# xUhEngwAng/I2V-Adapter-Unofficial

Measured on AMD Instinct MI355X. Metric: denoising steps/sec @ 16fx512x512 SD1.5+I2V-Adapter, higher is better.
Workload: dtype f16

## Files before the change

i2v-adapter-unofficial_amd/_lib.py:

```python
import ctypes as C
import os

_HERE = os.path.dirname(os.path.abspath(__file__))
LIB_PATH = os.environ.get("I2V_LIB_PATH") or os.path.join(_HERE, "libi2v_hip.so")
ABI_VERSION = 28

I2V_EPI_NONE, I2V_EPI_GELU, I2V_EPI_GEGLU = 0, 1, 2
I2V_STORE_ROWMAJOR, I2V_STORE_ROWPERM, I2V_STORE_VT, I2V_STORE_VT_T = 0, 1, 2, 3
I2V_A_PLAIN, I2V_A_CONV3X3 = 0, 1
I2V_LORA_MAX_ADAPTERS, I2V_LORA_MAX_RANK = 8, 256
I2V_ROUTE_GENERIC, I2V_ROUTE_CONV_THIN, I2V_ROUTE_BIG_TILE, I2V_ROUTE_BIG_DEEP, I2V_ROUTE_BIG_SPLITK = 0, 1, 2, 3, 4
I2V_EXTRA_NONE, I2V_EXTRA_LNF, I2V_EXTRA_HILO, I2V_EXTRA_GNS, I2V_EXTRA_UPF = 0, 1, 2, 4, 8
I2V_TATTN_LDS_FORM, I2V_TATTN_REG_FORM = 0, 1
I2V_ADD_RES_MAX = 16
I2V_TAESD_PREP_IDENTITY, I2V_TAESD_PREP_UNIT, I2V_TAESD_PREP_CLAMP = 0, 1, 2


class HipLibraryError(RuntimeError):
    pass


class GemmParams(C.Structure):
    _fields_ = [
        ("a", C.c_void_p), ("lda", C.c_int64),
        ("a2", C.c_void_p), ("lda2", C.c_int64),
        ("k_split", C.c_int32), ("a_mode", C.c_int32),
        ("w", C.c_void_p), ("ldw", C.c_int64),
        ("bias", C.c_void_p),
# ... 223 lines not shown
    "i2v_gemm_f16": (C.c_int, [C.POINTER(GemmParams), _P]),
    "i2v_gemm_ln_supported": (C.c_int, [C.POINTER(GemmParams)]),
    "i2v_gemm_batch_supported": (C.c_int, [C.POINTER(GemmParams)]),
    "i2v_gemm_upconv_fold_supported": (C.c_int, [C.POINTER(GemmParams)]),
    "i2v_gemm_workspace_bytes": (C.c_int64, [C.POINTER(GemmParams)]),
    "i2v_gemm_gn_partial_rows": (C.c_int32, [C.POINTER(GemmParams)]),
    "i2v_gemm_route": (C.c_int, [C.POINTER(GemmParams), C.POINTER(GemmRoute)]),
    "i2v_gemm_last_route": (C.c_int, [C.POINTER(GemmRoute)]),
    "i2v_gemm_kernel_exists": (C.c_int, [C.POINTER(GemmRoute)]),
    "i2v_attention_f16": (C.c_int, [C.POINTER(AttnParams), _P]),
    "i2v_temporal_attention_f16": (C.c_int, [C.POINTER(TAttnParams), _P]),
    "i2v_temporal_attention_route": (C.c_int, [C.POINTER(TAttnParams), C.POINTER(TAttnRoute)]),
    "i2v_temporal_attention_last_route": (C.c_int, [C.POINTER(TAttnRoute)]),
    "i2v_tattn_kernel_exists": (C.c_int, [C.POINTER(TAttnRoute)]),
    "i2v_motion_attn_supported": (C.c_int32, [C.c_int64, C.c_int32, C.c_int32, C.c_int32, C.c_int32]),
    "i2v_motion_attn_pack_rows": (C.c_int32, [C.c_int32, C.c_int32]),
    "i2v_motion_attn_f16": (C.c_int, [C.POINTER(MotionAttnParams), _P]),
    "i2v_motion_attn_wide_supported": (C.c_int32, [C.c_int64, C.c_int32, C.c_int32, C.c_int32, C.c_int32]),
    "i2v_motion_attn_wide_f16": (C.c_int, [C.POINTER(MotionAttnParams), _P]),
    "i2v_cross_attn_fused_supported": (C.c_int32, [C.c_int64, C.c_int32, C.c_int32, C.c_int32, C.c_int32, C.c_int64]),
    "i2v_cross_attn_fused_pack_rows": (C.c_int32, [C.c_int32, C.c_int32]),
    "i2v_cross_attn_fused_ctx_elems": (C.c_int64, [C.c_int32, C.c_int32, C.c_int32]),
    "i2v_cross_attn_fused_f16": (C.c_int, [C.POINTER(CrossAttnFusedParams), _P]),
    "i2v_ln_qkv_supported": (C.c_int32, [C.c_int64, C.c_int32, C.c_int32, C.c_int64]),
    "i2v_ln_qkv_f16": (C.c_int, [C.POINTER(LnQkvParams), _P]),
    "i2v_ff_fused_supported": (C.c_int32, [C.c_int64, C.c_int32, C.c_int32]),
    "i2v_ff_fused_tail_supported": (C.c_int32, [C.c_int64, C.c_int32, C.c_int32, C.c_int32, C.c_int32]),
    "i2v_ff_fused_f16": (C.c_int, [C.POINTER(FfFusedParams), _P]),
    "i2v_groupnorm_workspace_bytes": (C.c_int64, [C.c_int32, C.c_int32, C.c_int32]),
    "i2v_groupnorm_f16": (C.c_int, [C.POINTER(GnParams), _P]),
    "i2v_groupnorm_fold_f16": (C.c_int, [C.POINTER(GnParams), _P, C.c_int64, _P, C.c_int32, _P, _P, _P]),
    "i2v_layernorm_f16": (C.c_int, [C.POINTER(LnParams), _P]),
    "i2v_softmax_rows_f16": (C.c_int, [_P, C.c_int64, _P, C.c_int64, C.c_int32, C.c_int32, C.c_float, _P]),
    "i2v_nchw_to_tokens": (C.c_int, [_P, C.c_int32, _P, C.c_int32, C.c_int32, C.c_int32, C.c_int32, _P]),
    "i2v_tokens_to_nchw": (C.c_int, [_P, C.c_int32, C.c_int64, _P, C.c_int32, C.c_int32, C.c_int32, C.c_int32, _P]),
    "i2v_timestep_embedding": (C.c_int, [_P, _P, C.c_int32, _P, C.c_int32, C.c_int32, _P]),
    "i2v_silu_f16": (C.c_int, [_P, _P, C.c_int64, _P]),
    "i2v_repeat_rows_f16": (C.c_int, [_P, _P, C.c_int64, C.c_int64, C.c_int32, _P]),
    "i2v_copy3d_f16": (C.c_int, [_P, C.c_int64, C.c_int64, _P, C.c_int64, C.c_int64, C.c_int64, C.c_int64,
                                 C.c_int64, _P]),
    "i2v_pack_ctx_fragments_elems": (C.c_int64, [C.c_int32, C.c_int32, C.c_int32]),
    "i2v_pack_ctx_fragments_f16": (C.c_int, [_P, C.c_int64, _P, C.c_int64, C.c_int64, _P, C.c_int32, C.c_int32, C.c_int32, C.c_int32, _P]),
    "i2v_ddim_prep": (C.c_int, [_P, _P, _P, C.c_int32, C.c_int32, C.c_int32, C.c_int32, C.c_int32, C.c_int32, _P]),
    "i2v_gaussian_sample_f32": (C.c_int, [_P, _P, _P, C.c_int32, C.c_int32, C.c_int32, _P]),
    "i2v_first_frame_prior_f32": (C.c_int, [_P, _P, _P, _P, C.c_int32, C.c_int32, C.c_int32, C.c_int32, C.c_int32,
                                            C.c_float, C.c_float, C.c_float, C.c_float, C.c_float, _P]),
# ... 120 lines not shown
```

i2v-adapter-unofficial_amd/csrc/handle.hip:

```cpp
#include <string.h>

#include <map>
#include <string>
#include <vector>

#include "common.h"

namespace {

constexpr uint32_t PLAN_MAGIC = 0x50563249u;
constexpr uint32_t PLAN_VERSION = 1;
struct PlanHeader {
  uint32_t magic, version, abi, n_ops, n_keys, n_relocs;
  int32_t batch, frames, height, width, ctx_len, has_ip;
  uint64_t arena_bytes;
  uint32_t io_read_mask, reserved;
  uint64_t keys_off, ops_off, relocs_off, payload_off, payload_bytes, total_bytes;
};
struct PlanOp {
  uint32_t entry, payload_off, payload_bytes, reloc_begin, reloc_count, struct_bytes;
};
struct PlanReloc {
  uint32_t offset, kind, index, pad;
  uint64_t addend;
};
enum { RELOC_ARENA = 0, RELOC_WEIGHT = 1, RELOC_IO = 2 };

enum Entry {
  E_GEMM = 0, E_ATTN, E_TATTN, E_MOTION_ATTN, E_CROSS_ATTN_FUSED, E_LN_QKV, E_FF_FUSED, E_GROUPNORM, E_LAYERNORM,
  E_GROUPNORM_FOLD, E_NCHW_TO_TOKENS, E_TOKENS_TO_NCHW, E_TIMESTEP_EMBEDDING, E_SILU, E_REPEAT_ROWS, E_COPY3D, E_SELECT_ROW,
  E_PACK_CTX_FRAGMENTS, E_DDIM_PREP, E_DDIM_CFG_STEP, E_DPM_CFG_STEP, E_FREEU, E_LCM_CFG_STEP, E_FREENOISE_GATHER,
  E_FREENOISE_BLEND, E_MOTION_ATTN_WIDE, E_COUNT
};
struct EntryInfo {
  const char* name;
  uint32_t struct_bytes;
  uint32_t slots;
};
const EntryInfo ENTRIES[E_COUNT] = {
    {"i2v_gemm_f16", sizeof(i2v_gemm_params), 0},
    {"i2v_attention_f16", sizeof(i2v_attn_params), 0},
    {"i2v_temporal_attention_f16", sizeof(i2v_tattn_params), 0},
    {"i2v_motion_attn_f16", sizeof(i2v_motion_attn_params), 0},
    {"i2v_cross_attn_fused_f16", sizeof(i2v_cross_attn_fused_params), 0},
    {"i2v_ln_qkv_f16", sizeof(i2v_ln_qkv_params), 0},
    {"i2v_ff_fused_f16", sizeof(i2v_ff_fused_params), 0},
    {"i2v_groupnorm_f16", sizeof(i2v_gn_params), 0},
    {"i2v_layernorm_f16", sizeof(i2v_ln_params), 0},
    {"i2v_groupnorm_fold_f16", sizeof(i2v_gn_params), 6},
    {"i2v_nchw_to_tokens", 0, 7},
    {"i2v_tokens_to_nchw", 0, 8},
    {"i2v_timestep_embedding", 0, 6},
    {"i2v_silu_f16", 0, 3},
    {"i2v_repeat_rows_f16", 0, 5},
    {"i2v_copy3d_f16", 0, 9},
    {"i2v_select_row_f16", 0, 6},
    {"i2v_pack_ctx_fragments_f16", 0, 10},
    {"i2v_ddim_prep", 0, 9},
    {"i2v_ddim_cfg_step", 0, 13},
    {"i2v_dpm_cfg_step", 0, 14},
    {"i2v_freeu_f16", 0, 13},
    {"i2v_lcm_cfg_step", 0, 15},
    {"i2v_freenoise_gather_f16", 0, 10},
    {"i2v_freenoise_blend_f16", 0, 12},
    {"i2v_motion_attn_wide_f16", sizeof(i2v_motion_attn_params), 0},
};
inline uint32_t pad8(uint32_t n) { return (n + 7u) & ~7u; }

}

struct i2v_unet {
  i2v_unet_config cfg;
  struct weight { const void* ptr; int32_t dtype, ndim; int64_t shape[4]; };
  std::map<std::string, weight> weights;
  uint64_t weights_generation = 0;
  i2v_unet_plan_t plan;
  bool planned = false;
  std::vector<unsigned char> blob;
  std::vector<std::string> keys;
  std::vector<const void*> key_ptr;
  uint64_t bound_generation = ~0ull;
  void* arena = nullptr;
  int64_t arena_bytes = 0;
  hipStream_t capture_stream = nullptr;
  bool capturing = false;
  hipGraph_t graph = nullptr;
  hipGraphExec_t exec = nullptr;

// ... 302 lines not shown
      case E_DPM_CFG_STEP:
        rc = i2v_dpm_cfg_step(reinterpret_cast<float*>(P(0)), reinterpret_cast<float*>(P(1)), P(2), (int32_t)I(3), I(4),
                              reinterpret_cast<const float*>(P(5)), (int32_t)I(6), reinterpret_cast<int32_t*>(P(7)), F(8), (int32_t)I(9),
                              (int32_t)I(10), (int32_t)I(11), (int32_t)I(12), (int32_t)I(13), stream);
        break;
      case E_FREEU:
        rc = i2v_freeu_f16(P(0), P(1), P(2), P(3), P(4), P(5), (int32_t)I(6), (int32_t)I(7), (int32_t)I(8), (int32_t)I(9), (int32_t)I(10), F(11),
                           F(12), stream);
        break;
      case E_LCM_CFG_STEP:
        rc = i2v_lcm_cfg_step(reinterpret_cast<float*>(P(0)), reinterpret_cast<const float*>(P(1)), (int32_t)I(2), P(3), (int32_t)I(4), I(5),
                              reinterpret_cast<const float*>(P(6)), (int32_t)I(7), reinterpret_cast<int32_t*>(P(8)), F(9), (int32_t)I(10),
                              (int32_t)I(11), (int32_t)I(12), (int32_t)I(13), (int32_t)I(14), stream);
        break;
      case E_FREENOISE_GATHER:
        rc = i2v_freenoise_gather_f16(P(0), I(1), P(2), I(3), reinterpret_cast<const int32_t*>(P(4)), I(5), (int32_t)I(6), (int32_t)I(7),
                                      (int32_t)I(8), (int32_t)I(9), stream);
        break;
      case E_FREENOISE_BLEND:
        rc = i2v_freenoise_blend_f16(P(0), I(1), P(2), I(3), reinterpret_cast<const int32_t*>(P(4)), reinterpret_cast<const float*>(P(5)), I(6),
                                     (int32_t)I(7), (int32_t)I(8), (int32_t)I(9), (int32_t)I(10), (int32_t)I(11), stream);
        break;
      case E_MOTION_ATTN_WIDE: rc = i2v_motion_attn_wide_f16(reinterpret_cast<const i2v_motion_attn_params*>(buf), stream); break;
      default: I2V_FAIL(I2V_ERR_UNSUPPORTED, "i2v_unet_forward: launch %u names entry point %u", i, op.entry);
    }
    if (rc != I2V_OK) return rc;
  }
  return I2V_OK;
}

extern "C" int i2v_unet_capture_step(i2v_unet* h, i2v_stream_t stream) {
  I2V_CHECK_ARG(h != nullptr && stream != nullptr, "i2v_unet_capture_step: null handle or the null stream (capture needs a stream of its own)");
  I2V_CHECK_ARG(h->planned, "i2v_unet_capture_step: i2v_unet_plan first");
  I2V_CHECK_ARG(!h->capturing, "i2v_unet_capture_step: a capture is already in progress (i2v_unet_abort_capture discards it)");
  drop_step(h);
  hipStream_t s = reinterpret_cast<hipStream_t>(stream);
  const hipError_t e = hipStreamBeginCapture(s, hipStreamCaptureModeRelaxed);
  if (e != hipSuccess) {
    (void)hipGetLastError();
    I2V_FAIL(I2V_ERR_LAUNCH, "i2v_unet_capture_step: hipStreamBeginCapture: %s", hipGetErrorString(e));
  }
  h->capture_stream = s;
  h->capturing = true;
  return I2V_OK;
}

// ... 30 lines not shown
```

i2v-adapter-unofficial_amd/csrc/motion_attn.hip:

```cpp
#include <stdlib.h>

#include <type_traits>

#include "common.h"

namespace {

__device__ __forceinline__ f32x4 mfma16x16x16(f16x4 a, f16x4 b, f32x4 c) {
  return __builtin_amdgcn_mfma_f32_16x16x16f16(a, b, c, 0, 0, 0);
}

__device__ __forceinline__ void ma_dma16(__amdgpu_buffer_rsrc_t rsrc, f16* lds_wave_base, unsigned voff, unsigned soff) {
  __builtin_amdgcn_raw_ptr_buffer_load_lds(rsrc, (__attribute__((address_space(3))) void*)lds_wave_base, 16, voff, soff, 0, 0);
}
__device__ __forceinline__ int ma_opaque(int v) {
  asm volatile("" : "+v"(v));
  return v;
}

constexpr int MA_PIX = 8;
constexpr int MA_F = 16;
constexpr int MA_PD = 3;
constexpr int MA_AD = 4;

// ... 1 lines not shown
  const void* x; int64_t ldx;
  const void* gamma; const void* shift; int64_t ld_shift;
  const void* w;
  void* out; int64_t ldo;
  float eps;
  const void* ctx_frag;
  int32_t lt; int32_t tiles_per_ctx;
  const void* ip_frag; int32_t ip_len; float ip_scale;
  const void* w_o; const void* b_o;
};

constexpr int MA_KT = 5;

template <int C, int D, int H, bool CROSS, int F = 16, bool OUTP = false, int PIX = MA_PIX>
__global__ __launch_bounds__(64 * H) void motion_attn_kernel(const ma_args p, const float scale_log2, const int ntiles,
                                                             long long* __restrict__ stamps) {
  constexpr int DT = (D + 15) / 16, DP = 16 * DT, KS = C / 32, NJ = C / 64, PARTS = CROSS ? 1 : 3;
  constexpr int RW = PIX * MA_F / H, HALVES = RW / 8;
  static_assert(C % 64 == 0 && H == 8, "one wave per head, 8 lanes x C / 64 chunks per row in the LayerNorm pass");
  static_assert(F == 8 || F == 16 || F == 32, "frames per pixel");
  static_assert(RW % 8 == 0 && PIX % (F == 32 ? 2 : 1) == 0, "whole groups of 8 rows per wave, whole pixels per tile");
  extern __shared__ __attribute__((aligned(16))) f16 panels[];
  const int tid = threadIdx.x, lane = tid & 63, wave = __builtin_amdgcn_readfirstlane(tid >> 6);
  const int g = lane >> 4, l15 = lane & 15, sub = lane & 7;
  const f16* __restrict__ X = reinterpret_cast<const f16*>(p.x);
  const float* __restrict__ gamma = reinterpret_cast<const float*>(p.gamma);
  const float* __restrict__ shift = reinterpret_cast<const float*>(p.shift);
#ifdef I2V_MA_STAMPS
  long long stamp[8];
#define MA_STAMP(k) stamp[k] = __builtin_amdgcn_s_memtime()
#else
#define MA_STAMP(k)
#endif

  auto fetch_rows = [&](const int tile, f16* panel) {
    const f16* base = X + ((int64_t)tile * (PIX * MA_F) + RW * wave) * p.ldx;
    const auto rs = __builtin_amdgcn_make_buffer_rsrc(const_cast<f16*>(base), 0, (int)(((RW - 1) * p.ldx + C) * 2), 0x00020000);
    const int ln = ma_opaque(lane);
    const unsigned voff = (unsigned)(((ln >> 3) * p.ldx + (ln & 7) * 8) * 2);
#pragma unroll
    for (int half = 0; half < HALVES; ++half)
#pragma unroll
      for (int j = 0; j < NJ; ++j)
        ma_dma16(rs, panel + RW * wave * C + (half * NJ + j) * 512, voff, (unsigned)((8 * half * p.ldx + 8 * j * 8) * 2));
  };
  constexpr bool LATE_TABLES = NJ > 5;
  auto normalise_rows = [&](f16* panel) {
    f16x8 xv[HALVES][NJ];
#pragma unroll
    for (int half = 0; half < HALVES; ++half)
#pragma unroll
      for (int j = 0; j < NJ; ++j) xv[half][j] = *reinterpret_cast<const f16x8*>(panel + RW * wave * C + ((half * NJ + j) * 64 + lane) * 8);
    const float* gp = gamma;
    const float* sp = shift;
    asm volatile("" : "+s"(gp), "+s"(sp));
    f32x4 ga[NJ][2];
    if constexpr (!LATE_TABLES) {
#pragma unroll
      for (int j = 0; j < NJ; ++j) {
        ga[j][0] = *reinterpret_cast<const f32x4*>(gp + (sub + 8 * j) * 8);
        ga[j][1] = *reinterpret_cast<const f32x4*>(gp + (sub + 8 * j) * 8 + 4);
      }
    }
#pragma unroll
    for (int half = 0; half < HALVES; ++half) {
      const int row = RW * wave + 8 * half + (lane >> 3);
      const float* sh = sp + (int64_t)((RW * wave + 8 * half + (lane >> 3)) & (F - 1)) * p.ld_shift;
      f32x4 sv[NJ][2];
      if constexpr (!LATE_TABLES) {
#pragma unroll
// ... 18 lines not shown
      for (int j = 0; j < NJ; ++j)
#pragma unroll
        for (int e = 0; e < 8; ++e) {
          v[j][e] -= mean;
          q = fmaf(v[j][e], v[j][e], q);
        }
      q = sum_lanes8(q);
      const float rstd = rsqrtf(q / (float)C + p.eps);
#pragma unroll
      for (int j = 0; j < NJ; ++j) {
        const int ch = sub + 8 * j;
        if constexpr (LATE_TABLES) {
          ga[j][0] = *reinterpret_cast<const f32x4*>(gp + ch * 8);
          ga[j][1] = *reinterpret_cast<const f32x4*>(gp + ch * 8 + 4);
          sv[j][0] = *reinterpret_cast<const f32x4*>(sh + ch * 8);
          sv[j][1] = *reinterpret_cast<const f32x4*>(sh + ch * 8 + 4);
        }
        f16x8 o;
#pragma unroll
        for (int e = 0; e < 8; ++e) o[e] = (f16)fmaf(v[j][e] * rstd, ga[j][e >> 2][e & 3], sv[j][e >> 2][e & 3]);
        *reinterpret_cast<f16x8*>(panel + row * C + ((ch ^ (row & 7)) * 8)) = o;
      }
    }
  };

  const auto rs_w = __builtin_amdgcn_make_buffer_rsrc(const_cast<void*>(p.w), 0, H * PARTS * DP * C * 2, 0x00020000);
  const int w_lane = lane * 16, w_wave = wave * (PARTS * DP * C * 2);
  const int sw = l15 & 7;
  const int swz[2] = {(g ^ sw) * 8, ((4 + g) ^ sw) * 8};
  f32x4 acc[PIX][DT];
  auto zero_init = [](const int, const int) { return f32x4{0.f, 0.f, 0.f, 0.f}; };
  auto no_hook = []() {};
  auto project = [&](const f16* panel, const __amdgpu_buffer_rsrc_t rs, const int wp, auto transposed, auto init, auto hook) {
    constexpr bool TR = decltype(transposed)::value;
    auto ldw = [&](const int s, const int t) {
      return __builtin_bit_cast(f16x8, __builtin_amdgcn_raw_buffer_load_b128(rs, w_lane, wp + (s * DT + t) * 1024, 0));
    };
    const f16* alane = panel + l15 * C;
    f16x8 wf[MA_PD][DT];
#pragma unroll
    for (int pix = 0; pix < PIX; ++pix)
#pragma unroll
      for (int t = 0; t < DT; ++t) acc[pix][t] = init(pix, t);
#pragma unroll
    for (int s = 0; s < MA_PD - 1; ++s)
#pragma unroll
// ... 126 lines not shown
      __builtin_amdgcn_sched_barrier(0);
    }

    f16x4 qh[PIX][DT];
    project(panel, rs_w, w_wave, std::true_type{}, zero_init, no_hook);
#pragma unroll
    for (int pix = 0; pix < PIX; ++pix)
#pragma unroll
      for (int t = 0; t < DT; ++t) qh[pix][t] = to_half(CROSS ? acc[pix][t] * scale_log2 : acc[pix][t]);
    MA_STAMP(3);
    if constexpr (CROSS && OUTP) lds_barrier();

    if constexpr (CROSS) {
      const int ctx = tile / p.tiles_per_ctx;
      const f16* cf = reinterpret_cast<const f16*>(p.ctx_frag) + ((int64_t)ctx * H + wave) * (2 * MA_KT * DT * 256) + lane * 4;
      f16x4 kf[MA_KT][DT], vf[DT][MA_KT];
#pragma unroll
      for (int kt = 0; kt < MA_KT; ++kt)
#pragma unroll
        for (int t = 0; t < DT; ++t) {
          kf[kt][t] = *reinterpret_cast<const f16x4*>(cf + (kt * DT + t) * 256);
          vf[t][kt] = *reinterpret_cast<const f16x4*>(cf + (MA_KT * DT + t * MA_KT + kt) * 256);
        }
      const bool has_ip = p.ip_len > 0;
      f16x4 kfi[DT], vfi[DT];
      if (has_ip) {
        const f16* ci = reinterpret_cast<const f16*>(p.ip_frag) + ((int64_t)ctx * H + wave) * (2 * MA_KT * DT * 256) + lane * 4;
#pragma unroll
        for (int t = 0; t < DT; ++t) {
          kfi[t] = *reinterpret_cast<const f16x4*>(ci + t * 256);
          vfi[t] = *reinterpret_cast<const f16x4*>(ci + (MA_KT * DT + t * MA_KT) * 256);
        }
      }
      MA_STAMP(4);
      MA_STAMP(5);
      f16* __restrict__ O = reinterpret_cast<f16*>(p.out) + (int64_t)tile * (PIX * MA_F) * p.ldo + wave * D;
      const int sln = ma_opaque(lane), sg = sln >> 4, sl15 = sln & 15;
#pragma unroll
      for (int pix = 0; pix < PIX; ++pix) {
        float sv[MA_KT][4];
        float mx = -INFINITY;
#pragma unroll
        for (int kt = 0; kt < MA_KT; ++kt) {
          f32x4 sacc = {0.f, 0.f, 0.f, 0.f};
#pragma unroll
          for (int t = 0; t < DT; ++t) sacc = mfma16x16x16(kf[kt][t], qh[pix][t], sacc);
#pragma unroll
          for (int r = 0; r < 4; ++r) {
            const bool live = (kt < MA_KT - 1 && p.lt > 16 * (MA_KT - 1)) || 16 * kt + 4 * g + r < p.lt;
            sv[kt][r] = live ? sacc[r] : -INFINITY;
            mx = fmaxf(mx, sv[kt][r]);
          }
        }
        mx = lane_xor32_max(lane_xor16_max(mx));
        float ls = 0.f;
#pragma unroll
        for (int kt = 0; kt < MA_KT; ++kt)
#pragma unroll
          for (int r = 0; r < 4; ++r) {
            sv[kt][r] = __builtin_amdgcn_exp2f(sv[kt][r] - mx);
            ls += sv[kt][r];
          }
        ls = lane_xor32_sum(lane_xor16_sum(ls));
        const float inv = 1.0f / ls;
        f16x4 pk[MA_KT];
#pragma unroll
        for (int kt = 0; kt < MA_KT; ++kt) pk[kt] = f16x4{(f16)sv[kt][0], (f16)sv[kt][1], (f16)sv[kt][2], (f16)sv[kt][3]};
        f32x4 ov[DT];
#pragma unroll
        for (int t = 0; t < DT; ++t) {
          f32x4 o = {0.f, 0.f, 0.f, 0.f};
#pragma unroll
          for (int kt = 0; kt < MA_KT; ++kt) o = mfma16x16x16(vf[t][kt], pk[kt], o);
          ov[t] = o * inv;
        }
        if (has_ip) {
          f32x4 sacc = {0.f, 0.f, 0.f, 0.f};
#pragma unroll
          for (int t = 0; t < DT; ++t) sacc = mfma16x16x16(kfi[t], qh[pix][t], sacc);
          float si[4];
          float mi = -INFINITY;
#pragma unroll
          for (int r = 0; r < 4; ++r) {
            si[r] = (4 * g + r < p.ip_len) ? sacc[r] : -INFINITY;
            mi = fmaxf(mi, si[r]);
          }
          mi = lane_xor32_max(lane_xor16_max(mi));
          float li = 0.f;
#pragma unroll
          for (int r = 0; r < 4; ++r) {
            si[r] = __builtin_amdgcn_exp2f(si[r] - mi);
            li += si[r];
          }
          li = lane_xor32_sum(lane_xor16_sum(li));
          const float wi = p.ip_scale / li;
          const f16x4 pi = {(f16)si[0], (f16)si[1], (f16)si[2], (f16)si[3]};
#pragma unroll
          for (int t = 0; t < DT; ++t) ov[t] += mfma16x16x16(vfi[t], pi, f32x4{0.f, 0.f, 0.f, 0.f}) * wi;
        }
// ... 171 lines not shown
  I2V_CHECK_ARG(p.w_o && p.b_o, "i2v_motion_attn_wide_f16: w_o and b_o are required (this form exists only with the out-projection inside)");
  I2V_CHECK_ARG(i2v_motion_attn_wide_supported(p.rows, p.channels, p.heads, p.head_dim, p.frames),
                "i2v_motion_attn_wide_f16: rows %lld channels %d heads %d head_dim %d frames %d is not a fused shape "
                "(i2v_motion_attn_wide_supported)", (long long)p.rows, p.channels, p.heads, p.head_dim, p.frames);
  I2V_CHECK_ARG(p.ldx >= p.channels && p.ldx % 8 == 0 && p.ldo >= p.channels && p.ldo % 8 == 0 && p.ld_shift >= p.channels &&
                p.ld_shift % 4 == 0, "i2v_motion_attn_wide_f16: row strides");
  I2V_CHECK_ARG(i2v_al16(p.x) && i2v_al16(p.gamma) && i2v_al16(p.shift) && i2v_al16(p.w_qkv) && i2v_al16(p.out) && i2v_al16(p.w_o) &&
                i2v_al16(p.b_o), "i2v_motion_attn_wide_f16: pointers must be 16-byte aligned");
  I2V_CHECK_ARG(p.ldx < (1 << 23), "i2v_motion_attn_wide_f16: ldx (%lld) must be below 2^23", (long long)p.ldx);
  ma_args a = {};
  a.x = p.x; a.ldx = p.ldx; a.gamma = p.gamma; a.shift = p.shift; a.ld_shift = p.ld_shift; a.w = p.w_qkv; a.out = p.out;
  a.ldo = p.ldo; a.eps = p.eps; a.w_o = p.w_o; a.b_o = p.b_o;
  return launch_ma<640, 80, 8, false, 16, true, MA_WIDE_PIX>(a, p.rows, p.scale, reinterpret_cast<hipStream_t>(stream),
                                                              "i2v_motion_attn_wide_f16");
}

extern "C" int32_t i2v_cross_attn_fused_supported(int64_t rows, int32_t channels, int32_t heads, int32_t head_dim, int32_t ctx_len,
                                                  int64_t rows_per_ctx) {
  return rows > 0 && rows % (MA_PIX * MA_F) == 0 && rows / (MA_PIX * MA_F) < (1 << 24) && channels == 320 && heads == 8 &&
         head_dim == 40 && ctx_len >= 1 && ctx_len <= 16 * MA_KT && rows_per_ctx > 0 && rows_per_ctx % (MA_PIX * MA_F) == 0 &&
         rows % rows_per_ctx == 0 && ma_cus<320, 40, 8, true>() > 0;
}

extern "C" int32_t i2v_cross_attn_fused_pack_rows(int32_t heads, int32_t head_dim) { return heads * ((head_dim + 15) / 16) * 16; }

extern "C" int64_t i2v_cross_attn_fused_ctx_elems(int32_t n_ctx, int32_t heads, int32_t head_dim) {
  return (int64_t)n_ctx * heads * 2 * MA_KT * ((head_dim + 15) / 16) * 256;
}

extern "C" int i2v_cross_attn_fused_f16(const i2v_cross_attn_fused_params* pp, i2v_stream_t stream) {
  I2V_CHECK_ARG(pp != nullptr, "i2v_cross_attn_fused_f16: null params");
  const i2v_cross_attn_fused_params& p = *pp;
  I2V_CHECK_ARG(p.x && p.gamma && p.beta && p.w_q && p.ctx_frag && p.out, "i2v_cross_attn_fused_f16: null pointer");
  I2V_CHECK_ARG(i2v_cross_attn_fused_supported(p.rows, p.channels, p.heads, p.head_dim, p.ctx_len, p.rows_per_ctx),
                "i2v_cross_attn_fused_f16: rows %lld channels %d heads %d head_dim %d ctx_len %d rows_per_ctx %lld is not a fused shape "
                "(i2v_cross_attn_fused_supported)", (long long)p.rows, p.channels, p.heads, p.head_dim, p.ctx_len,
                (long long)p.rows_per_ctx);
  I2V_CHECK_ARG(p.ldx >= p.channels && p.ldx % 8 == 0 && p.ldo >= p.channels && p.ldo % 8 == 0, "i2v_cross_attn_fused_f16: row strides");
  I2V_CHECK_ARG(i2v_al16(p.x) && i2v_al16(p.gamma) && i2v_al16(p.beta) && i2v_al16(p.w_q) && i2v_al16(p.out) && i2v_al16(p.ctx_frag) && i2v_al16(p.ip_frag),
                "i2v_cross_attn_fused_f16: pointers must be 16-byte aligned");
  I2V_CHECK_ARG(p.ip_frag == nullptr || (p.ip_len >= 1 && p.ip_len <= 16), "i2v_cross_attn_fused_f16: ip_len (%d) must be in [1, 16]",
                p.ip_len);
  ma_args a = {};
  a.x = p.x; a.ldx = p.ldx; a.gamma = p.gamma; a.shift = p.beta; a.ld_shift = 0; a.w = p.w_q; a.out = p.out; a.ldo = p.ldo;
  a.eps = p.eps;
  a.ctx_frag = p.ctx_frag; a.lt = p.ctx_len;
  a.ip_frag = p.ip_frag; a.ip_len = p.ip_frag ? p.ip_len : 0; a.ip_scale = p.ip_scale;
  a.tiles_per_ctx = (int32_t)(p.rows_per_ctx / (MA_PIX * MA_F));
  I2V_CHECK_ARG(p.w_o == nullptr || p.ldx < (1 << 23), "i2v_cross_attn_fused_f16: ldx (%lld) must be below 2^23 with the out-projection", (long long)p.ldx);
  I2V_CHECK_ARG((p.w_o == nullptr) == (p.b_o == nullptr) && i2v_al16(p.w_o) && i2v_al16(p.b_o),
                "i2v_cross_attn_fused_f16: w_o and b_o come together, 16-byte aligned");
  a.w_o = p.w_o; a.b_o = p.b_o;
  if (p.w_o != nullptr)
    return launch_ma<320, 40, 8, true, 16, true>(a, p.rows, p.scale, reinterpret_cast<hipStream_t>(stream), "i2v_cross_attn_fused_f16");
  return launch_ma<320, 40, 8, true>(a, p.rows, p.scale, reinterpret_cast<hipStream_t>(stream), "i2v_cross_attn_fused_f16");
}
```

i2v-adapter-unofficial_amd/handle.py:

```python
import bisect
import ctypes as C
import struct

import torch

from . import _lib

PLAN_MAGIC, PLAN_VERSION = 0x50563249, 1
ENTRY_IDS = {name: i for i, name in enumerate((
    "i2v_gemm_f16", "i2v_attention_f16", "i2v_temporal_attention_f16", "i2v_motion_attn_f16", "i2v_cross_attn_fused_f16", "i2v_ln_qkv_f16",
    "i2v_ff_fused_f16", "i2v_groupnorm_f16", "i2v_layernorm_f16", "i2v_groupnorm_fold_f16", "i2v_nchw_to_tokens", "i2v_tokens_to_nchw",
    "i2v_timestep_embedding", "i2v_silu_f16", "i2v_repeat_rows_f16", "i2v_copy3d_f16", "i2v_select_row_f16",
    "i2v_pack_ctx_fragments_f16", "i2v_ddim_prep", "i2v_ddim_cfg_step", "i2v_dpm_cfg_step"))}
LATER_ENTRY_IDS = {name: len(ENTRY_IDS) + i for i, name in enumerate((
    "i2v_freeu_f16",
    "i2v_lcm_cfg_step",
    "i2v_freenoise_gather_f16", "i2v_freenoise_blend_f16",
    "i2v_motion_attn_wide_f16"))}
ENTRY_NAMES = {i: n for n, i in {**ENTRY_IDS, "i2v_freeu_f16": LATER_ENTRY_IDS["i2v_freeu_f16"]}.items()}


def entry_id(name):
    return ENTRY_IDS.get(name, LATER_ENTRY_IDS.get(name))


def entry_name(i):
    return next((n for n, j in {**ENTRY_IDS, **LATER_ENTRY_IDS}.items() if j == i), None)


IO_SAMPLE, IO_TIMESTEPS, IO_CONTEXT, IO_IMAGE_EMBEDS, IO_OUT = range(5)
RELOC_ARENA, RELOC_WEIGHT, RELOC_IO = range(3)
_INT_TYPES = (C.c_int32, C.c_int64, C.c_int)


def _pad8(n):
    return (n + 7) & ~7


class _RecordingLib:

    def __init__(self, real):
# ... 517 lines not shown
```

i2v-adapter-unofficial_amd/i2v_adapter.py:

```python
import os
from typing import Optional

import torch
from torch import nn

from . import kernels as K
from . import streams
from .blocks import (gn_proj_in, ff_tail_operands, precise_stream, Attention, FeedForward, HipModule, LazyPack, LnFoldPlan, _as_f16_matrix,
                     fold_layernorm, from_tokens, to_tokens, w16)
from ._lib import HipLibraryError
from .checkpoint import PretrainedMixin

f16 = torch.float16


def get_block(out_channel, block_depth, num_attention_heads, transformer_layers_per_block):
    block = nn.Module()
    attn_blocks = []
    for _ in range(block_depth):
        attn_block = nn.Module()
        tbs = []
        for _ in range(transformer_layers_per_block):
            tb = nn.Module()
            tb.i2v_adapter = Attention(query_dim=out_channel, heads=num_attention_heads,
# ... 11 lines not shown
    def __init__(self, block_depth, block_out_channels, num_attention_heads,
                 transformer_layers_per_block: int = 1, mid_block_depth: int = 1):
        super().__init__()
        self.config = dict(block_depth=block_depth, block_out_channels=tuple(block_out_channels),
                           num_attention_heads=num_attention_heads,
                           transformer_layers_per_block=transformer_layers_per_block,
                           mid_block_depth=mid_block_depth)
        self.down_blocks = nn.ModuleList([
            get_block(c, block_depth, num_attention_heads, transformer_layers_per_block)
            for c in block_out_channels[:-1]])
        rev = list(reversed(block_out_channels[:-1]))
        up_blocks = nn.ModuleList([
            get_block(c, block_depth + 1, num_attention_heads, transformer_layers_per_block) for c in rev])
        self.up_blocks = nn.ModuleList([nn.Identity()]) + up_blocks
        self.mid_block = get_block(block_out_channels[-1], mid_block_depth, num_attention_heads,
                                   transformer_layers_per_block)

    def forward(self):
        pass


FUSED_TEXT_ATTN = os.environ.get("I2V_TEXT_FUSED", "1") != "0"
FUSED_ATTN_OUT = os.environ.get("I2V_ATTN_OUTP", "1") != "0"
FUSED_LN_QKV = os.environ.get("I2V_QKV_FUSED", "1") != "0"


class I2VAdapterTransformerBlock(HipModule):

    def __init__(self, dim: int, num_attention_heads: int, attention_head_dim: int, dropout=0.0,
                 cross_attention_dim: Optional[int] = None, activation_fn: str = "geglu",
                 num_embeds_ada_norm: Optional[int] = None, attention_bias: bool = False,
                 only_cross_attention: bool = False, double_self_attention: bool = False,
                 upcast_attention: bool = False, norm_elementwise_affine: bool = True,
                 norm_type: str = "layer_norm", norm_eps: float = 1e-5, final_dropout: bool = False,
                 attention_type: str = "default", positional_embeddings: Optional[str] = None,
                 num_positional_embeddings: Optional[int] = None, ff_inner_dim: Optional[int] = None,
                 ff_bias: bool = True, attention_out_bias: bool = True, with_adapter: bool = True, **_unused):
        super().__init__()
        if norm_type != "layer_norm" or only_cross_attention or double_self_attention or positional_embeddings:
            raise NotImplementedError("only the layer-norm spatial block of the hot path is implemented "
                                      "(SURVEY 8b: ada-norm / GLIGEN / only_cross_attention branches are dropped)")
        self.dim, self.heads, self.dim_head = dim, num_attention_heads, attention_head_dim
        self.eps = norm_eps
        self.only_cross_attention = only_cross_attention
        self.norm1 = nn.LayerNorm(dim, elementwise_affine=norm_elementwise_affine, eps=norm_eps)
        self.attn1 = Attention(query_dim=dim, heads=num_attention_heads, dim_head=attention_head_dim,
# ... 132 lines not shown
            x = K.gemm(o1, p["w_o_dual"], p["b_o_dual"], a2=o2, residual=x)
        else:
            x = K.gemm(o1, p["w_o1"], p["b_o1"], residual=x)
        if cfg_expand:
            x, n_img = K.duplicate_batch(x), 2 * n_img
        if self.attn2 is not None:
            if ctx_text is None:
                raise ValueError("encoder_hidden_states is required by the cross-attention layer")
            if n_img % ctx_text.shape[0] != 0:
                raise ValueError(f"context batch {ctx_text.shape[0]} does not divide batch {n_img}")
            kv_group = n_img // ctx_text.shape[0]
            kv = self.attn2.context_kv(ctx_text, ctx_ip)
            _k, _vt, kip, _vtip, lt, li = kv
            use_ip = kip is not None and bool(self.attn2.ip_num_tokens)
            fused_out2 = False
            if FUSED_TEXT_ATTN and (not use_ip or li <= 16) and \
                    K.cross_attn_fused_supported(x.shape[0], c, self.heads, self.dim_head, lt, kv_group * L):
                frag, frag_ip = self.attn2.context_fragments(ctx_text, kv)
                o = K.cross_attn_fused(x, p["g2_f32"], p["b2_f32"], p["wq2_frag"], frag, heads=self.heads, head_dim=self.dim_head,
                                       ctx_len=lt, rows_per_ctx=kv_group * L, eps=self.eps, scale=self.attn2.scale,
                                       ip_frag=frag_ip, ip_len=li if use_ip else 0, ip_scale=float(self.attn2.ip_scale),
                                       out_proj=p["wo2_frag"] if FUSED_ATTN_OUT else None)
                fused_out2 = FUSED_ATTN_OUT
            else:
                if fold2:
                    wf, ws, cb = p["f_q2"]
                    q = K.gemm(x, wf, cb, ln=(ws, self.eps))
                else:
                    n = K.layernorm(x, p["g2"], p["b2"], self.eps)
                    q = K.gemm(n, p["w_q2"])
                o = self.attn2._cross(q, ctx_text, ctx_ip, n_img, L, kv_group, kv=kv)
            if fused_out2:
                x = o
            else:
                x = K.gemm(o, p["w_o2"], p["b_o2"], residual=x)
        def ret(v, applied=False):
            return v if tail is None else (v, applied)
        if self.ff.fused_supported(x):
            if self.ff.tail_supported(x, tail):
                return ret(self.ff._fwd_fused(x, p["g3_f32"], p["b3_f32"], self.eps, tail=tail), True)
            return ret(self.ff._fwd_fused(x, p["g3_f32"], p["b3_f32"], self.eps))
        if fold3:
            return ret(self.ff._fwd_folded(x, self.eps, p["f_ff"]))
        n = K.layernorm(x, p["g3"], p["b3"], self.eps)
        return ret(self.ff._fwd(n, x))

# ... 132 lines not shown
```

i2v-adapter-unofficial_amd/kernels.py:

```python
import ctypes as C
import functools
import os
from typing import Optional

import torch

from . import _lib
from ._lib import (I2V_A_CONV3X3, I2V_A_PLAIN, I2V_EPI_GEGLU, I2V_EPI_GELU, I2V_EPI_NONE, I2V_STORE_ROWMAJOR,
                   I2V_STORE_ROWPERM, I2V_STORE_VT, I2V_STORE_VT_T, AttnBwdParams, AttnParams, GemmParams, GnParams,
                   HipLibraryError, LnParams, TAttnParams)

f16 = torch.float16


def _stream():
    return C.c_void_p(torch.cuda.current_stream().cuda_stream)


def _req(t: torch.Tensor, name: str, dtype=f16):
    if not isinstance(t, torch.Tensor):
        raise TypeError(f"{name} must be a tensor")
    if not t.is_cuda:
        raise HipLibraryError(f"{name} is on {t.device}: the I2V-Adapter HIP path has no CPU fallback "
                              "(move tensors to a ROCm device)")
# ... 512 lines not shown
    if out is None:
        out = torch.empty(shape, dtype=f16, device=k.device)
    elif tuple(out.shape) != shape or out.dtype != f16 or not out.is_contiguous():
        raise ValueError(f"pack_ctx_fragments: out is {tuple(out.shape)}, expected {shape}")
    _lib.check(lib.i2v_pack_ctx_fragments_f16(_p(k), ldk, _p(vt), vt.stride(1), vt.stride(0), _p(out), n_ctx, heads, d, ctx_len,
                                              _stream()), "i2v_pack_ctx_fragments_f16")
    return out


def pack_attn_out(w_o, b_o, heads):
    return pack_cross_q(w_o, heads), b_o.detach().float().contiguous()


def _attn_out_operands(out_proj, c, heads, head_dim, what):
    w_o, b_o = out_proj
    _req(w_o, "w_o")
    _req(b_o, "b_o", dtype=torch.float32)
    if tuple(w_o.shape) != (_lib.load().i2v_cross_attn_fused_pack_rows(heads, head_dim), c) or not w_o.is_contiguous() or \
            b_o.numel() != c or not b_o.is_contiguous():
        raise ValueError(f"{what}: out_proj is {tuple(w_o.shape)} / {tuple(b_o.shape)} (pack_attn_out)")
    return _p(w_o), _p(b_o)


def cross_attn_fused(x, gamma32, beta32, w_q, ctx_frag, *, heads, head_dim, ctx_len, rows_per_ctx, eps, scale=None, out=None,
                     ip_frag=None, ip_len=0, ip_scale=1.0, out_proj=None):
    lib = _lib.load()
    x, ldx = _mat(x, "x")
    rows, c = x.shape
    _req(w_q, "w_q")
    _req(ctx_frag, "ctx_frag")
    for name, t in (("gamma32", gamma32), ("beta32", beta32)):
        _req(t, name, dtype=torch.float32)
        if tuple(t.shape) != (c,):
            raise ValueError(f"cross_attn_fused: {name} is {tuple(t.shape)}, expected ({c},)")
    n_ctx = -(-rows // rows_per_ctx)
    if c != heads * head_dim or not ctx_frag.is_contiguous() or \
            ctx_frag.numel() != lib.i2v_cross_attn_fused_ctx_elems(n_ctx, heads, head_dim):
        raise ValueError(f"cross_attn_fused: ctx_frag is {tuple(ctx_frag.shape)} for {n_ctx} contexts (pack_ctx_fragments)")
    if tuple(w_q.shape) != (lib.i2v_cross_attn_fused_pack_rows(heads, head_dim), c) or not w_q.is_contiguous():
        raise ValueError(f"cross_attn_fused: w_q is {tuple(w_q.shape)} (pack_cross_q)")
    if out is None:
        out = torch.empty((rows, c), dtype=f16, device=x.device)
    out, ldo = _mat(out, "out")
    p = _lib.CrossAttnFusedParams()
    p.x, p.ldx = _p(x), ldx
    p.gamma, p.beta, p.w_q = _p(gamma32), _p(beta32), _p(w_q)
    p.ctx_frag = _p(ctx_frag)
    p.out, p.ldo = _p(out), ldo
    p.rows, p.rows_per_ctx = rows, rows_per_ctx
    p.channels, p.heads, p.head_dim, p.ctx_len = c, heads, head_dim, ctx_len
    p.eps, p.scale = float(eps), float(head_dim) ** -0.5 if scale is None else float(scale)
    if ip_frag is not None:
        _req(ip_frag, "ip_frag")
        if not ip_frag.is_contiguous() or ip_frag.numel() != ctx_frag.numel():
            raise ValueError(f"cross_attn_fused: ip_frag is {tuple(ip_frag.shape)} (pack_ctx_fragments of the image tokens)")
        p.ip_frag, p.ip_len, p.ip_scale = _p(ip_frag), int(ip_len), float(ip_scale)
    if out_proj is not None:
        p.w_o, p.b_o = _attn_out_operands(out_proj, c, heads, head_dim, "cross_attn_fused")
    _lib.check(lib.i2v_cross_attn_fused_f16(C.byref(p), _stream()), "i2v_cross_attn_fused_f16")
    return out


def ln_qkv_supported(rows, channels, n_qk, rows_per_image):
    return bool(_lib.load().i2v_ln_qkv_supported(rows, channels, n_qk, rows_per_image))


def pack_ln_qkv(w_qk, w_v):
    w = torch.cat([w_qk.detach().to(f16), w_v.detach().to(f16)], dim=0)
    n, c = w.shape
    if n % 160 or c % 32:
        raise ValueError(f"pack_ln_qkv: {n} rows x {c} columns is not whole waves of 160 rows / K steps of 32")
    return w.view(n // 16, 16, c // 32, 4, 8).permute(0, 2, 3, 1, 4).contiguous().view(n, c)


def ln_qkv(x, gamma32, beta32, w_packed, *, n_qk, rows_per_image, eps, qk=None, vt=None, images=None, x_image_stride=0):
    lib = _lib.load()
    x, ldx = _mat(x, "x")
    rows, c = x.shape
    if images is not None:
        if x_image_stride % ldx or (images - 1) * (x_image_stride // ldx) + rows_per_image > rows:
            raise ValueError(f"ln_qkv: {images} images of {rows_per_image} rows at stride {x_image_stride} do not fit x {tuple(x.shape)}")
        rows = images * rows_per_image
# ... 1339 lines not shown
```

include/i2v_hip.h:

```cpp
#ifndef I2V_HIP_H
#define I2V_HIP_H

#include <stdint.h>

#ifdef __cplusplus
extern "C" {
#endif

#define I2V_ABI_VERSION 28

#define I2V_OK 0
#define I2V_ERR_INVALID_ARG (-1)
#define I2V_ERR_UNSUPPORTED (-2)
#define I2V_ERR_LAUNCH (-3)

typedef void* i2v_stream_t;

int i2v_abi_version(void);
const char* i2v_last_error(void);

enum {
  I2V_EPI_NONE = 0,
  I2V_EPI_GELU = 1,
  I2V_EPI_GEGLU = 2
};

enum {
  I2V_STORE_ROWMAJOR = 0,
  I2V_STORE_ROWPERM = 1,
  I2V_STORE_VT = 2,
  I2V_STORE_VT_T = 3
};
// ... 134 lines not shown

int32_t i2v_motion_attn_wide_supported(int64_t rows, int32_t channels, int32_t heads, int32_t head_dim, int32_t frames);
int i2v_motion_attn_wide_f16(const i2v_motion_attn_params* p, i2v_stream_t stream);

typedef struct i2v_cross_attn_fused_params {
  const void* x; int64_t ldx;
  const void* gamma; const void* beta;
  const void* w_q;
  const void* ctx_frag;
  void* out; int64_t ldo;
  int64_t rows, rows_per_ctx;
  int32_t channels, heads, head_dim, ctx_len;
  float eps, scale;
  const void* ip_frag; int32_t ip_len; float ip_scale;
  const void* w_o; const void* b_o;
} i2v_cross_attn_fused_params;

int32_t i2v_cross_attn_fused_supported(int64_t rows, int32_t channels, int32_t heads, int32_t head_dim, int32_t ctx_len,
                                       int64_t rows_per_ctx);
int32_t i2v_cross_attn_fused_pack_rows(int32_t heads, int32_t head_dim);
int64_t i2v_cross_attn_fused_ctx_elems(int32_t n_ctx, int32_t heads, int32_t head_dim);
int i2v_cross_attn_fused_f16(const i2v_cross_attn_fused_params* p, i2v_stream_t stream);

typedef struct i2v_ln_qkv_params {
  const void* x; int64_t ldx;
  const void* gamma; const void* beta;
  const void* w;
  void* qk; int64_t ld_qk;
  void* vt; int64_t vt_batch_stride, vt_row_stride;
  int64_t rows, rows_per_image;
  int32_t channels, n_qk;
  float eps;
  int64_t x_image_stride;
} i2v_ln_qkv_params;

int32_t i2v_ln_qkv_supported(int64_t rows, int32_t channels, int32_t n_qk, int64_t rows_per_image);
int i2v_ln_qkv_f16(const i2v_ln_qkv_params* p, i2v_stream_t stream);

typedef struct i2v_ff_fused_params {
  const void* x; int64_t ldx;
  const void* gamma; const void* beta;
  const void* w1; const void* b1;
  const void* w2; const void* b2;
  void* out; int64_t ldo;
  int64_t rows;
  int32_t channels, inner;
// ... 288 lines not shown
```

Measured before the change: 21.91.

## Add wide fused cross-attention kernel for 640-channel blocks with out-projection

Adds a wide variant of the fused LayerNorm+Q-projection+cross-attention+out-projection kernel, instantiated for 640 channels, 8 heads and head_dim 80, reusing the wide motion-attention template. It covers the mid-resolution transformer blocks, which previously fell back to separate norm, GEMM and attention launches. Supporting template changes load image-prompt fragments late, zero padded V lanes, and use an opaque lane index to limit register pressure when DT>3. This adds kernel complexity and register pressure in exchange for fewer launches and less intermediate memory traffic.

```diff
diff --git a/i2v-adapter-unofficial_amd/_lib.py b/i2v-adapter-unofficial_amd/_lib.py
--- a/i2v-adapter-unofficial_amd/_lib.py
+++ b/i2v-adapter-unofficial_amd/_lib.py
@@ -3,7 +3,7 @@
 
 _HERE = os.path.dirname(os.path.abspath(__file__))
 LIB_PATH = os.environ.get("I2V_LIB_PATH") or os.path.join(_HERE, "libi2v_hip.so")
-ABI_VERSION = 28
+ABI_VERSION = 29
 
 I2V_EPI_NONE, I2V_EPI_GELU, I2V_EPI_GEGLU = 0, 1, 2
 I2V_STORE_ROWMAJOR, I2V_STORE_ROWPERM, I2V_STORE_VT, I2V_STORE_VT_T = 0, 1, 2, 3
@@ -273,6 +273,8 @@
     "i2v_cross_attn_fused_pack_rows": (C.c_int32, [C.c_int32, C.c_int32]),
     "i2v_cross_attn_fused_ctx_elems": (C.c_int64, [C.c_int32, C.c_int32, C.c_int32]),
     "i2v_cross_attn_fused_f16": (C.c_int, [C.POINTER(CrossAttnFusedParams), _P]),
+    "i2v_cross_attn_fused_wide_supported": (C.c_int32, [C.c_int64, C.c_int32, C.c_int32, C.c_int32, C.c_int32, C.c_int64]),
+    "i2v_cross_attn_fused_wide_f16": (C.c_int, [C.POINTER(CrossAttnFusedParams), _P]),
     "i2v_ln_qkv_supported": (C.c_int32, [C.c_int64, C.c_int32, C.c_int32, C.c_int64]),
     "i2v_ln_qkv_f16": (C.c_int, [C.POINTER(LnQkvParams), _P]),
     "i2v_ff_fused_supported": (C.c_int32, [C.c_int64, C.c_int32, C.c_int32]),
diff --git a/i2v-adapter-unofficial_amd/csrc/handle.hip b/i2v-adapter-unofficial_amd/csrc/handle.hip
--- a/i2v-adapter-unofficial_amd/csrc/handle.hip
+++ b/i2v-adapter-unofficial_amd/csrc/handle.hip
@@ -30,7 +30,7 @@
   E_GEMM = 0, E_ATTN, E_TATTN, E_MOTION_ATTN, E_CROSS_ATTN_FUSED, E_LN_QKV, E_FF_FUSED, E_GROUPNORM, E_LAYERNORM,
   E_GROUPNORM_FOLD, E_NCHW_TO_TOKENS, E_TOKENS_TO_NCHW, E_TIMESTEP_EMBEDDING, E_SILU, E_REPEAT_ROWS, E_COPY3D, E_SELECT_ROW,
   E_PACK_CTX_FRAGMENTS, E_DDIM_PREP, E_DDIM_CFG_STEP, E_DPM_CFG_STEP, E_FREEU, E_LCM_CFG_STEP, E_FREENOISE_GATHER,
-  E_FREENOISE_BLEND, E_MOTION_ATTN_WIDE, E_COUNT
+  E_FREENOISE_BLEND, E_MOTION_ATTN_WIDE, E_CROSS_ATTN_FUSED_WIDE, E_COUNT
 };
 struct EntryInfo {
   const char* name;
@@ -64,6 +64,7 @@
     {"i2v_freenoise_gather_f16", 0, 10},
     {"i2v_freenoise_blend_f16", 0, 12},
     {"i2v_motion_attn_wide_f16", sizeof(i2v_motion_attn_params), 0},
+    {"i2v_cross_attn_fused_wide_f16", sizeof(i2v_cross_attn_fused_params), 0},
 };
 inline uint32_t pad8(uint32_t n) { return (n + 7u) & ~7u; }
 
@@ -412,6 +413,9 @@
                                      (int32_t)I(7), (int32_t)I(8), (int32_t)I(9), (int32_t)I(10), (int32_t)I(11), stream);
         break;
       case E_MOTION_ATTN_WIDE: rc = i2v_motion_attn_wide_f16(reinterpret_cast<const i2v_motion_attn_params*>(buf), stream); break;
+      case E_CROSS_ATTN_FUSED_WIDE:
+        rc = i2v_cross_attn_fused_wide_f16(reinterpret_cast<const i2v_cross_attn_fused_params*>(buf), stream);
+        break;
       default: I2V_FAIL(I2V_ERR_UNSUPPORTED, "i2v_unet_forward: launch %u names entry point %u", i, op.entry);
     }
     if (rc != I2V_OK) return rc;
diff --git a/i2v-adapter-unofficial_amd/csrc/motion_attn.hip b/i2v-adapter-unofficial_amd/csrc/motion_attn.hip
--- a/i2v-adapter-unofficial_amd/csrc/motion_attn.hip
+++ b/i2v-adapter-unofficial_amd/csrc/motion_attn.hip
@@ -47,7 +47,7 @@
   static_assert(RW % 8 == 0 && PIX % (F == 32 ? 2 : 1) == 0, "whole groups of 8 rows per wave, whole pixels per tile");
   extern __shared__ __attribute__((aligned(16))) f16 panels[];
   const int tid = threadIdx.x, lane = tid & 63, wave = __builtin_amdgcn_readfirstlane(tid >> 6);
-  const int g = lane >> 4, l15 = lane & 15, sub = lane & 7;
+  const int g = lane >> 4, l15 = lane & 15;
   const f16* __restrict__ X = reinterpret_cast<const f16*>(p.x);
   const float* __restrict__ gamma = reinterpret_cast<const float*>(p.gamma);
   const float* __restrict__ shift = reinterpret_cast<const float*>(p.shift);
@@ -70,7 +70,8 @@
         ma_dma16(rs, panel + RW * wave * C + (half * NJ + j) * 512, voff, (unsigned)((8 * half * p.ldx + 8 * j * 8) * 2));
   };
   constexpr bool LATE_TABLES = NJ > 5;
-  auto normalise_rows = [&](f16* panel) {
+  auto normalise_rows_as = [&](f16* panel, auto redo) {
+    const int lane = decltype(redo)::value ? ma_opaque(tid) & 63 : tid & 63, sub = lane & 7;
     f16x8 xv[HALVES][NJ];
 #pragma unroll
     for (int half = 0; half < HALVES; ++half)
@@ -135,6 +136,10 @@
         *reinterpret_cast<f16x8*>(panel + row * C + ((ch ^ (row & 7)) * 8)) = o;
       }
     }
+  };
+
+  auto normalise_rows = [&](f16* panel) {
+    normalise_rows_as(panel, std::bool_constant<CROSS && LATE_TABLES>{});
   };
 
   const auto rs_w = __builtin_amdgcn_make_buffer_rsrc(const_cast<void*>(p.w), 0, H * PARTS * DP * C * 2, 0x00020000);
@@ -307,9 +312,10 @@
           kf[kt][t] = *reinterpret_cast<const f16x4*>(cf + (kt * DT + t) * 256);
           vf[t][kt] = *reinterpret_cast<const f16x4*>(cf + (MA_KT * DT + t * MA_KT + kt) * 256);
         }
+      constexpr bool IP_LATE = DT > 3;
       const bool has_ip = p.ip_len > 0;
       f16x4 kfi[DT], vfi[DT];
-      if (has_ip) {
+      if (!IP_LATE && has_ip) {
         const f16* ci = reinterpret_cast<const f16*>(p.ip_frag) + ((int64_t)ctx * H + wave) * (2 * MA_KT * DT * 256) + lane * 4;
 #pragma unroll
         for (int t = 0; t < DT; ++t) {
@@ -321,6 +327,19 @@
       MA_STAMP(5);
       f16* __restrict__ O = reinterpret_cast<f16*>(p.out) + (int64_t)tile * (PIX * MA_F) * p.ldo + wave * D;
       const int sln = ma_opaque(lane), sg = sln >> 4, sl15 = sln & 15;
+      constexpr bool CLEAR_PAD = DT > 3;
+      auto clear_pad = [](f16x4& v, const int live) {
+        u32x2 b = __builtin_bit_cast(u32x2, v);
+        b[0] &= live >= 2 ? 0xffffffffu : live == 1 ? 0x0000ffffu : 0u;
+        b[1] &= live >= 4 ? 0xffffffffu : live == 3 ? 0x0000ffffu : 0u;
+        v = __builtin_bit_cast(f16x4, b);
+      };
+      if constexpr (CLEAR_PAD) {
+#pragma unroll
+        for (int kt = 0; kt < MA_KT; ++kt)
+#pragma unroll
+          for (int t = 0; t < DT; ++t) clear_pad(vf[t][kt], p.lt - 16 * kt - 4 * sg);
+      }
 #pragma unroll
       for (int pix = 0; pix < PIX; ++pix) {
         float sv[MA_KT][4];
@@ -360,6 +379,15 @@
           ov[t] = o * inv;
         }
         if (has_ip) {
+          if constexpr (IP_LATE) {
+            const f16* ci = reinterpret_cast<const f16*>(p.ip_frag) + ((int64_t)ctx * H + wave) * (2 * MA_KT * DT * 256) + ma_opaque(lane) * 4;
+#pragma unroll
+            for (int t = 0; t < DT; ++t) {
+              kfi[t] = *reinterpret_cast<const f16x4*>(ci + t * 256);
+              vfi[t] = *reinterpret_cast<const f16x4*>(ci + (MA_KT * DT + t * MA_KT) * 256);
+              clear_pad(vfi[t], p.ip_len - 4 * sg);
+            }
+          }
           f32x4 sacc = {0.f, 0.f, 0.f, 0.f};
 #pragma unroll
           for (int t = 0; t < DT; ++t) sacc = mfma16x16x16(kfi[t], qh[pix][t], sacc);
@@ -577,6 +605,13 @@
          rows % rows_per_ctx == 0 && ma_cus<320, 40, 8, true>() > 0;
 }
 
+extern "C" int32_t i2v_cross_attn_fused_wide_supported(int64_t rows, int32_t channels, int32_t heads, int32_t head_dim, int32_t ctx_len,
+                                                       int64_t rows_per_ctx) {
+  return rows > 0 && rows % (MA_WIDE_PIX * MA_F) == 0 && rows / (MA_WIDE_PIX * MA_F) < (1 << 24) && channels == 640 && heads == 8 &&
+         head_dim == 80 && ctx_len >= 1 && ctx_len <= 16 * MA_KT && rows_per_ctx > 0 && rows_per_ctx % (MA_WIDE_PIX * MA_F) == 0 &&
+         rows % rows_per_ctx == 0 && ma_cus<640, 80, 8, true, 16, true, MA_WIDE_PIX>() > 0;
+}
+
 extern "C" int32_t i2v_cross_attn_fused_pack_rows(int32_t heads, int32_t head_dim) { return heads * ((head_dim + 15) / 16) * 16; }
 
 extern "C" int64_t i2v_cross_attn_fused_ctx_elems(int32_t n_ctx, int32_t heads, int32_t head_dim) {
@@ -610,3 +645,29 @@
     return launch_ma<320, 40, 8, true, 16, true>(a, p.rows, p.scale, reinterpret_cast<hipStream_t>(stream), "i2v_cross_attn_fused_f16");
   return launch_ma<320, 40, 8, true>(a, p.rows, p.scale, reinterpret_cast<hipStream_t>(stream), "i2v_cross_attn_fused_f16");
 }
+
+extern "C" int i2v_cross_attn_fused_wide_f16(const i2v_cross_attn_fused_params* pp, i2v_stream_t stream) {
+  I2V_CHECK_ARG(pp != nullptr, "i2v_cross_attn_fused_wide_f16: null params");
+  const i2v_cross_attn_fused_params& p = *pp;
+  I2V_CHECK_ARG(p.x && p.gamma && p.beta && p.w_q && p.ctx_frag && p.out, "i2v_cross_attn_fused_wide_f16: null pointer");
+  I2V_CHECK_ARG(p.w_o && p.b_o, "i2v_cross_attn_fused_wide_f16: w_o and b_o are required (this form exists only with the out-projection inside)");
+  I2V_CHECK_ARG(i2v_cross_attn_fused_wide_supported(p.rows, p.channels, p.heads, p.head_dim, p.ctx_len, p.rows_per_ctx),
+                "i2v_cross_attn_fused_wide_f16: rows %lld channels %d heads %d head_dim %d ctx_len %d rows_per_ctx %lld is not a fused shape "
+                "(i2v_cross_attn_fused_wide_supported)", (long long)p.rows, p.channels, p.heads, p.head_dim, p.ctx_len,
+                (long long)p.rows_per_ctx);
+  I2V_CHECK_ARG(p.ldx >= p.channels && p.ldx % 8 == 0 && p.ldo >= p.channels && p.ldo % 8 == 0, "i2v_cross_attn_fused_wide_f16: row strides");
+  I2V_CHECK_ARG(i2v_al16(p.x) && i2v_al16(p.gamma) && i2v_al16(p.beta) && i2v_al16(p.w_q) && i2v_al16(p.out) && i2v_al16(p.ctx_frag) &&
+                i2v_al16(p.ip_frag) && i2v_al16(p.w_o) && i2v_al16(p.b_o), "i2v_cross_attn_fused_wide_f16: pointers must be 16-byte aligned");
+  I2V_CHECK_ARG(p.ip_frag == nullptr || (p.ip_len >= 1 && p.ip_len <= 16), "i2v_cross_attn_fused_wide_f16: ip_len (%d) must be in [1, 16]",
+                p.ip_len);
+  I2V_CHECK_ARG(p.ldx < (1 << 23), "i2v_cross_attn_fused_wide_f16: ldx (%lld) must be below 2^23", (long long)p.ldx);
+  ma_args a = {};
+  a.x = p.x; a.ldx = p.ldx; a.gamma = p.gamma; a.shift = p.beta; a.ld_shift = 0; a.w = p.w_q; a.out = p.out; a.ldo = p.ldo;
+  a.eps = p.eps;
+  a.ctx_frag = p.ctx_frag; a.lt = p.ctx_len;
+  a.ip_frag = p.ip_frag; a.ip_len = p.ip_frag ? p.ip_len : 0; a.ip_scale = p.ip_scale;
+  a.tiles_per_ctx = (int32_t)(p.rows_per_ctx / (MA_WIDE_PIX * MA_F));
+  a.w_o = p.w_o; a.b_o = p.b_o;
+  return launch_ma<640, 80, 8, true, 16, true, MA_WIDE_PIX>(a, p.rows, p.scale, reinterpret_cast<hipStream_t>(stream),
+                                                             "i2v_cross_attn_fused_wide_f16");
+}
diff --git a/i2v-adapter-unofficial_amd/handle.py b/i2v-adapter-unofficial_amd/handle.py
--- a/i2v-adapter-unofficial_amd/handle.py
+++ b/i2v-adapter-unofficial_amd/handle.py
@@ -16,7 +16,8 @@
     "i2v_freeu_f16",
     "i2v_lcm_cfg_step",
     "i2v_freenoise_gather_f16", "i2v_freenoise_blend_f16",
-    "i2v_motion_attn_wide_f16"))}
+    "i2v_motion_attn_wide_f16",
+    "i2v_cross_attn_fused_wide_f16"))}
 ENTRY_NAMES = {i: n for n, i in {**ENTRY_IDS, "i2v_freeu_f16": LATER_ENTRY_IDS["i2v_freeu_f16"]}.items()}
 
 
diff --git a/i2v-adapter-unofficial_amd/i2v_adapter.py b/i2v-adapter-unofficial_amd/i2v_adapter.py
--- a/i2v-adapter-unofficial_amd/i2v_adapter.py
+++ b/i2v-adapter-unofficial_amd/i2v_adapter.py
@@ -57,6 +57,7 @@
 
 FUSED_TEXT_ATTN = os.environ.get("I2V_TEXT_FUSED", "1") != "0"
 FUSED_ATTN_OUT = os.environ.get("I2V_ATTN_OUTP", "1") != "0"
+FUSED_TEXT_ATTN_WIDE = os.environ.get("I2V_TEXT_FUSED_WIDE", "1") != "0"
 FUSED_LN_QKV = os.environ.get("I2V_QKV_FUSED", "1") != "0"
 
 
@@ -235,6 +236,14 @@
                                        ip_frag=frag_ip, ip_len=li if use_ip else 0, ip_scale=float(self.attn2.ip_scale),
                                        out_proj=p["wo2_frag"] if FUSED_ATTN_OUT else None)
                 fused_out2 = FUSED_ATTN_OUT
+            elif FUSED_TEXT_ATTN and FUSED_ATTN_OUT and FUSED_TEXT_ATTN_WIDE and (not use_ip or li <= 16) and \
+                    K.cross_attn_fused_wide_supported(x.shape[0], c, self.heads, self.dim_head, lt, kv_group * L):
+                frag, frag_ip = self.attn2.context_fragments(ctx_text, kv)
+                o = K.cross_attn_fused_wide(x, p["g2_f32"], p["b2_f32"], p["wq2_frag"], frag, heads=self.heads, head_dim=self.dim_head,
+                                            ctx_len=lt, rows_per_ctx=kv_group * L, eps=self.eps, scale=self.attn2.scale,
+                                            ip_frag=frag_ip, ip_len=li if use_ip else 0, ip_scale=float(self.attn2.ip_scale),
+                                            out_proj=p["wo2_frag"])
+                fused_out2 = True
             else:
                 if fold2:
                     wf, ws, cb = p["f_q2"]
diff --git a/i2v-adapter-unofficial_amd/kernels.py b/i2v-adapter-unofficial_amd/kernels.py
--- a/i2v-adapter-unofficial_amd/kernels.py
+++ b/i2v-adapter-unofficial_amd/kernels.py
@@ -558,8 +558,21 @@
     return _p(w_o), _p(b_o)
 
 
+def cross_attn_fused_wide_supported(rows, channels, heads, head_dim, ctx_len, rows_per_ctx):
+    return bool(_lib.load().i2v_cross_attn_fused_wide_supported(rows, channels, heads, head_dim, ctx_len, rows_per_ctx))
+
+
+def cross_attn_fused_wide(x, gamma32, beta32, w_q, ctx_frag, *, heads, head_dim, ctx_len, rows_per_ctx, eps, out_proj, scale=None,
+                          out=None, ip_frag=None, ip_len=0, ip_scale=1.0):
+    if out_proj is None:
+        raise ValueError("cross_attn_fused_wide: out_proj is required (pack_attn_out)")
+    return cross_attn_fused(x, gamma32, beta32, w_q, ctx_frag, heads=heads, head_dim=head_dim, ctx_len=ctx_len, rows_per_ctx=rows_per_ctx,
+                            eps=eps, scale=scale, out=out, ip_frag=ip_frag, ip_len=ip_len, ip_scale=ip_scale, out_proj=out_proj,
+                            _entry="i2v_cross_attn_fused_wide_f16")
+
+
 def cross_attn_fused(x, gamma32, beta32, w_q, ctx_frag, *, heads, head_dim, ctx_len, rows_per_ctx, eps, scale=None, out=None,
-                     ip_frag=None, ip_len=0, ip_scale=1.0, out_proj=None):
+                     ip_frag=None, ip_len=0, ip_scale=1.0, out_proj=None, _entry="i2v_cross_attn_fused_f16"):
     lib = _lib.load()
     x, ldx = _mat(x, "x")
     rows, c = x.shape
@@ -593,7 +606,7 @@
         p.ip_frag, p.ip_len, p.ip_scale = _p(ip_frag), int(ip_len), float(ip_scale)
     if out_proj is not None:
         p.w_o, p.b_o = _attn_out_operands(out_proj, c, heads, head_dim, "cross_attn_fused")
-    _lib.check(lib.i2v_cross_attn_fused_f16(C.byref(p), _stream()), "i2v_cross_attn_fused_f16")
+    _lib.check(getattr(lib, _entry)(C.byref(p), _stream()), _entry)
     return out
 
 
diff --git a/include/i2v_hip.h b/include/i2v_hip.h
--- a/include/i2v_hip.h
+++ b/include/i2v_hip.h
@@ -7,7 +7,7 @@
 extern "C" {
 #endif
 
-#define I2V_ABI_VERSION 28
+#define I2V_ABI_VERSION 29
 
 #define I2V_OK 0
 #define I2V_ERR_INVALID_ARG (-1)
@@ -188,6 +188,10 @@
 int64_t i2v_cross_attn_fused_ctx_elems(int32_t n_ctx, int32_t heads, int32_t head_dim);
 int i2v_cross_attn_fused_f16(const i2v_cross_attn_fused_params* p, i2v_stream_t stream);
 
+int32_t i2v_cross_attn_fused_wide_supported(int64_t rows, int32_t channels, int32_t heads, int32_t head_dim, int32_t ctx_len,
+                                            int64_t rows_per_ctx);
+int i2v_cross_attn_fused_wide_f16(const i2v_cross_attn_fused_params* p, i2v_stream_t stream);
+
 typedef struct i2v_ln_qkv_params {
   const void* x; int64_t ldx;
   const void* gamma; const void* beta;
```

Result: no change. 21.85 (-0.3%).
